# LepistaBioinformatics/blutils

Measured on AMD Instinct MI355X. Metric: Mqueries/sec consensus (synthetic outfmt-6 hit table), higher is better.
Workload: dtype i32/u32

## Files before the change

### blutils_amd/csrc/consensus_kernel.hip

```cpp

#if defined(__HIP_DEVICE_COMPILE__) && !defined(__gfx950__)
#error "consensus_kernel.hip is written for gfx950"
#endif

#include <hip/hip_runtime.h>

#include <climits>
#include <cstdint>
#include <type_traits>

#include "blu_internal.h"

namespace blu {

#define WAVE 64

constexpr int BLOCK_A = 768;
constexpr int BLU_WAVES_PER_SIMD = 3;
constexpr int BLOCK_N = 1024;
constexpr int BLU_N_WAVES_PER_SIMD = 4;
constexpr int BLOCK_F = 704;
constexpr int LIST_CAP = 208;
constexpr int LIST_CAP_RING = 248;
constexpr int LIST_CAP_F64 = 232;
// ... 681 lines not shown
                else { m[0] = wave_max_i32(m[0]); m[1] = wave_max_i32(m[1]); }
                uint32_t c[2], slot[2], tot[2], tmask[2];
#pragma unroll
                for (int hf = 0; hf < 2; ++hf) {
                    c[hf] = 0; tmask[hf] = 0;
#pragma unroll
                    for (int r = 0; r < 4; ++r) { const bool t = left[hf] > r && bs[hf][r] == m[hf]; tmask[hf] |= (uint32_t)t << r; c[hf] += (uint32_t)t; }
                    uint32_t in = c[hf];
                    in += (uint32_t)dpp<0x111>((int)in);
                    in += (uint32_t)dpp<0x112>((int)in);
                    in += (uint32_t)dpp<0x114>((int)in);
                    in += (uint32_t)dpp<0x118>((int)in);
                    const uint32_t k0 = (uint32_t)rl((int)in, 15), k1 = (uint32_t)rl((int)in, 31), k2 = (uint32_t)rl((int)in, 47), k3 = (uint32_t)rl((int)in, 63);
                    tot[hf] = k0 + k1 + k2 + k3;
                    slot[hf] = (row16 == 0 ? 0u : (row16 == 1 ? k0 : (row16 == 2 ? k0 + k1 : k0 + k1 + k2))) + in - c[hf];
                }
                const uint32_t gk = tot[0] + tot[1];
                const bool fits = fill + gk <= CAP;
                if (lane == 0) {
                    if (halves) L.meta[qi] = fits ? (fill | (gk << 16)) : META_SLOW;
                    else {
                        L.meta[qs[0]] = fits ? (fill | (tot[0] << 16)) : META_SLOW;
                        if (qs[1] < 64u) L.meta[qs[1]] = fits ? ((fill + tot[0]) | (tot[1] << 16)) : META_SLOW;
                    }
                }
                if (!fits) {
                    uint64_t rest = long_mask;
                    while (rest) { const uint32_t qn = (uint32_t)__builtin_ctzll(rest); rest &= rest - 1; if (lane == 0) L.meta[qn] = META_SLOW; }
                    break;
                }
                {
#pragma unroll
                    for (int hf = 0; hf < 2; ++hf) {
                        if (tot[hf] == 0) continue;
                        StepRegs S;
                        fetch_rest(S, voff[hf], tmask[hf]);
                        uint32_t idx = fill + (hf ? tot[0] : 0u) + slot[hf];
#pragma unroll
                        for (int r = 0; r < 4; ++r) {
                            if ((tmask[hf] >> r) & 1u) {
                                put_entry(idx, S, r, ro[hf] + sub4 + r);
                                ++idx;
                            }
                        }
                    }
                    fill += gk;
                }
            }
        };
        auto phase1_flat = [&]() {
            if constexpr (!RING) {
            constexpr uint32_t UR = FLAT_ROWS, MAXS = FLAT_STEPS, DEPTH = FLAT_DEPTH;
            static_assert(UR == 8u, "two 16-byte loads per lane");
            static_assert(FLAT_SEG >= MAX_TASK_SEG, "the flat pass takes every segment of the task");
            static_assert(DEPTH <= MAXS && MAXS * WAVE >= FLAT_SEG / UR, "a query's units fit one round");
            const uint32_t rows = L.seg[lane].y;
            const uint32_t nunit = (rows + UR - 1u) / UR;
            uint32_t incl = nunit;
            incl += (uint32_t)dpp<0x111>((int)incl);
            incl += (uint32_t)dpp<0x112>((int)incl);
            incl += (uint32_t)dpp<0x114>((int)incl);
            incl += (uint32_t)dpp<0x118>((int)incl);
            const uint32_t t0 = (uint32_t)rl((int)incl, 15), t1 = (uint32_t)rl((int)incl, 31), t2 = (uint32_t)rl((int)incl, 47);
            const uint32_t r16 = (uint32_t)lane >> 4;
            incl += r16 == 0 ? 0u : (r16 == 1 ? t0 : (r16 == 2 ? t0 + t1 : t0 + t1 + t2));
            const uint32_t q_end = incl, q_begin = incl - nunit;
            const uint64_t out_m = __ballot(rows != 0u && q_end > MAXS * WAVE);
            const uint32_t q_lim = out_m ? (uint32_t)__builtin_ctzll(out_m) : WAVE;
            const uint32_t total = q_lim < WAVE ? (uint32_t)rl((int)q_begin, (int)q_lim) : (uint32_t)rl((int)q_end, WAVE - 1);
            const uint32_t ns = (total + WAVE - 1u) / WAVE;
            L.qs[lane] = q_begin;
            L.qm[lane] = INT_MIN;
            L.qk[lane] = 0u;
            if (rows != 0u) L.meta[lane] = META_SLOW;
            __builtin_amdgcn_fence(__ATOMIC_RELEASE, "workgroup");
            __builtin_amdgcn_wave_barrier();
            __builtin_amdgcn_fence(__ATOMIC_ACQUIRE, "workgroup");
            auto issue = [&](const uint32_t st, u32x4& lo4, u32x4& hi4, uint32_t& um) {
                um = 0u;
                uint32_t voff = 0xFFFFFFF0u;
                int left = 0;
                if (st < ns) {
                    const uint32_t g = st * WAVE + (uint32_t)lane;
                    uint32_t q = 0;
#pragma unroll
                    for (uint32_t sp = 32; sp; sp >>= 1) { const uint32_t c = q + sp; if (L.qs[c] <= g) q = c; }
                    const uint2 sg = L.seg[q];
                    const uint32_t oq = g - L.qs[q];
                    left = g < total ? (int)sg.y - (int)(UR * oq) : 0;
                    if (left > 0) { voff = (sg.x + UR * oq) * 4u; um = q | (oq << 6) | (umin((uint32_t)left, UR) << 12); }
                }
                lo4 = __builtin_amdgcn_raw_buffer_load_b128(rs_bs, voff, 0, STREAM_AUX);
                hi4 = __builtin_amdgcn_raw_buffer_load_b128(rs_bs, left > 4 ? voff + 16u : 0xFFFFFFF0u, 0, STREAM_AUX);
            };
            u32x4 ba[DEPTH], bb[DEPTH];
            uint32_t um[MAXS];
            int lmx[MAXS];
#pragma unroll
            for (uint32_t st = 0; st < MAXS; ++st) { um[st] = 0u; lmx[st] = INT_MIN; }
#pragma unroll
            for (uint32_t st = 0; st < DEPTH; ++st) issue(st, ba[st], bb[st], um[st]);
#pragma unroll
            for (uint32_t st = 0; st < MAXS; ++st) {
                if (st >= ns) break;
                const u32x4 va = ba[st % DEPTH], vb = bb[st % DEPTH];
                const uint32_t left = (um[st] >> 12) & 15u;
                const uint32_t v[8] = {va.x, va.y, va.z, va.w, vb.x, vb.y, vb.z, vb.w};
                int bsv[UR], mx = INT_MIN;
#pragma unroll
                for (uint32_t r = 0; r < UR; ++r) { bsv[r] = left > r ? (int)v[r] : INT_MIN; mx = imax(mx, bsv[r]); }
                uint32_t lmask = 0;
#pragma unroll
                for (uint32_t r = 0; r < UR; ++r) lmask |= (uint32_t)(left > r && bsv[r] == mx) << r;
                um[st] |= lmask << 16;
                lmx[st] = mx;
                if (left) atomicMax(&L.qm[um[st] & 63u], mx);
                if (st + DEPTH < MAXS) issue(st + DEPTH, ba[st % DEPTH], bb[st % DEPTH], um[st + DEPTH]);
            }
            __builtin_amdgcn_fence(__ATOMIC_RELEASE, "workgroup");
            __builtin_amdgcn_wave_barrier();
            __builtin_amdgcn_fence(__ATOMIC_ACQUIRE, "workgroup");
            uint32_t running = fill, q_cut = q_lim;
#pragma unroll
            for (uint32_t st = 0; st < MAXS; ++st) {
                if (st >= ns) break;
                const uint32_t q = um[st] & 63u, oq = (um[st] >> 6) & 63u;
                const bool have = ((um[st] >> 12) & 15u) != 0u;
                const int M = L.qm[q];
                const uint32_t tmask = (have && lmx[st] == M) ? (um[st] >> 16) & 0xFFu : 0u;
                const uint32_t c = (uint32_t)__builtin_popcount(tmask);
                uint32_t in2 = c;
                in2 += (uint32_t)dpp<0x111>((int)in2);
                in2 += (uint32_t)dpp<0x112>((int)in2);
                in2 += (uint32_t)dpp<0x114>((int)in2);
                in2 += (uint32_t)dpp<0x118>((int)in2);
                const uint32_t k0 = (uint32_t)rl((int)in2, 15), k1 = (uint32_t)rl((int)in2, 31), k2 = (uint32_t)rl((int)in2, 47), k3 = (uint32_t)rl((int)in2, 63);
                in2 += r16 == 0 ? 0u : (r16 == 1 ? k0 : (r16 == 2 ? k0 + k1 : k0 + k1 + k2));
                const uint32_t idx0 = running + in2 - c;
                if (have && oq == 0u) L.meta[q] = META_SLOW | idx0;
                if (c) atomicAdd(&L.qk[q], c);
                const bool over = have && idx0 + c > CAP;
                const uint64_t over_m = __ballot(over);
                const bool room = !over && c != 0u && (over_m == 0ull || (uint32_t)lane < (uint32_t)__builtin_ctzll(over_m));
                if (room) L.rec[idx0] = make_uint4(__builtin_bitreverse32(tmask), L.seg[q].x + UR * oq, UR * oq, 0u);
                if (over_m) { q_cut = (uint32_t)rl((int)q, __builtin_ctzll(over_m)); break; }
                running += k0 + k1 + k2 + k3;
            }
            __builtin_amdgcn_fence(__ATOMIC_RELEASE, "workgroup");
            __builtin_amdgcn_wave_barrier();
            __builtin_amdgcn_fence(__ATOMIC_ACQUIRE, "workgroup");
            const uint32_t m = L.meta[lane];
            if (rows != 0u && (uint32_t)lane < q_cut) L.meta[lane] = (m & 0xFFFFu) | (L.qk[lane] << 16);
            fill = q_cut < q_lim ? (L.meta[q_cut] & 0xFFFFu) : running;
            if (q_cut < WAVE) stop_q = q_cut;
            }
        };
        auto ring_mark_landed = [&](const uint32_t upto) {
            const uint32_t m0 = (ring_landed + RING_CHUNKS - 1u) & ~(RING_CHUNKS - 1u);
            if (m0 < upto) {
                if ((uint32_t)lane < RING_PAD) L.ring[RING_ROWS + lane] = L.ring[lane];
                __builtin_amdgcn_fence(__ATOMIC_RELEASE, "workgroup");
                __builtin_amdgcn_wave_barrier();
                __builtin_amdgcn_fence(__ATOMIC_ACQUIRE, "workgroup");
            }
            ring_landed = upto;
        };
        auto ring_refill = [&]() {
            if (ring_head < ring_tail) { ring_head = ring_tail; if (ring_landed < ring_tail) ring_landed = ring_tail; }
            const uint32_t lim = ring_end < ring_tail + RING_CHUNKS ? ring_end : ring_tail + RING_CHUNKS;
            if (ring_head < lim) { ring_dma_run(rs_ring, ring_c0, ring_head, lim); ring_head = lim; }
        };
        auto phase1_scan = [&](const auto rpl_c, const auto full_c, const uint32_t LPQ) {
            constexpr uint32_t RPL = decltype(rpl_c)::value;
            constexpr bool FULL = decltype(full_c)::value;
            static_assert(RPL <= RING_PAD && RPL <= 32u, "rows per lane");
            const uint32_t QPS = WAVE / LPQ;
            const uint32_t grp = (uint32_t)lane / LPQ, sub = ((uint32_t)lane & (LPQ - 1u)) * RPL, row16 = (uint32_t)lane >> 4;
            {
                const uint32_t cs = (uint32_t)((vbase + (uint32_t)rl((int)seg_x, (int)first_q)) >> 8);
                if (cs < ring_tail) { wait_vmcnt(0u); ring_head = ring_landed = ring_tail = cs; }
            }
            for (uint32_t qb = first_q / QPS * QPS; qb < nq; qb += QPS) {
                const uint32_t r_lo = (uint32_t)rl((int)seg_x, (int)(qb < first_q ? first_q : qb));
                const uint32_t qn = qb + QPS;
                const uint32_t r_hi = qn < nq ? (uint32_t)rl((int)seg_x, (int)qn) : task_nrows;
                ring_tail = (uint32_t)((vbase + r_lo) >> 8);
                ring_refill();
                if (r_hi > r_lo) {
                    const uint32_t need = (uint32_t)((vbase + r_hi - 1u) >> 8);
                    if (need >= ring_landed) { wait_vmcnt(ring_head - 1u - need); ring_mark_landed(need + 1u); }
                }
                const uint32_t qi = qb + grp;
                const uint2 sg = L.seg[qi];
                const int left0 = (sg.y > short_seg ? 0 : (int)sg.y) - (int)sub;
                const uint32_t over = (FULL && left0 > 0 && left0 < (int)RPL) ? RPL - (uint32_t)left0 : 0u;
                const uint32_t sub_e = sub - over;
                const int left = FULL ? (left0 > 0 ? (int)RPL : 0) : left0;
                const uint32_t row0 = sg.x + sub_e;
                const uint32_t a = ((uint32_t)vbase + sg.x + sub_e) & RING_MASK;
                int b[RPL];
#pragma unroll
                for (uint32_t i = 0; i < RPL; ++i) b[i] = (int)L.ring[a + i];
                asm volatile("s_waitcnt lgkmcnt(0)" ::: "memory");
#pragma unroll
                for (uint32_t i = 0; i < RPL; ++i) asm volatile("" : "+v"(b[i]));
                if (r_hi > r_lo) { ring_tail = (uint32_t)((vbase + r_hi) >> 8); ring_refill(); }
                int M = INT_MIN;
                if constexpr (FULL) {
#pragma unroll
                    for (uint32_t i = 0; i < RPL; ++i) M = imax(M, b[i]);
                    M = left > 0 ? M : INT_MIN;
                } else {
#pragma unroll
                    for (uint32_t i = 0; i < RPL; ++i) { b[i] = (int)i < left ? b[i] : INT_MIN; M = imax(M, b[i]); }
                }
                if (LPQ >= 2) M = imax(M, dpp<0xB1>(M));
                if (LPQ >= 4) M = imax(M, dpp<0x4E>(M));
                if (LPQ >= 8) M = imax(M, dpp<0x141>(M));
                if (LPQ >= 16) M = imax(M, dpp<0x140>(M));
                uint32_t mask = tie_mask<RPL>(b, M);
                mask = left > 0 ? mask : 0u;
                if constexpr (FULL) mask &= 0xFFFFFFFFu >> (32u - RPL + over);
                const uint32_t c = (uint32_t)__builtin_popcount(mask);
                uint32_t incl = c;
                incl += (uint32_t)dpp<0x111>((int)incl);
                incl += (uint32_t)dpp<0x112>((int)incl);
                incl += (uint32_t)dpp<0x114>((int)incl);
                incl += (uint32_t)dpp<0x118>((int)incl);
                const uint32_t k0 = (uint32_t)rl((int)incl, 15), k1 = (uint32_t)rl((int)incl, 31);
                const uint32_t k2 = (uint32_t)rl((int)incl, 47), k3 = (uint32_t)rl((int)incl, 63);
                const bool fits = fill + k0 + k1 + k2 + k3 <= CAP;
                const uint32_t p1 = fill + k0, p2 = p1 + k1, p3 = p2 + k2;
                const uint32_t rbase = row16 == 0 ? fill : (row16 == 1 ? p1 : (row16 == 2 ? p2 : p3));
                uint32_t gk = c;
                if (LPQ >= 2) gk += (uint32_t)dpp<0xB1>((int)gk);
                if (LPQ >= 4) gk += (uint32_t)dpp<0x4E>((int)gk);
                if (LPQ >= 8) gk += (uint32_t)dpp<0x141>((int)gk);
                if (LPQ >= 16) gk += (uint32_t)dpp<0x140>((int)gk);
                if (PID32 && !fits) {
                    __builtin_amdgcn_s_setprio(2);
                    uint64_t BK = 0;
                    uint32_t bacc = 0, bpos = 0, brow = 0, kmin = 0xFFFFFFFFu, pmax = 0, dlo = 0xFFFFFFFFu, dhi = 0, err = 0xFFFFFFFFu;
                    auto reset = [&]() { BK = 0; bacc = 0; bpos = 0; brow = 0; kmin = 0xFFFFFFFFu; pmax = 0; dlo = 0xFFFFFFFFu; dhi = 0; err = 0xFFFFFFFFu; };
                    auto better = [&](const uint64_t K, const uint32_t acc, const uint32_t pos, const uint64_t K2, const uint32_t acc2, const uint32_t pos2) {
                        const bool gt = (K > K2) | ((K == K2) & (acc > acc2)), eq = (K == K2) & (acc == acc2);
                        return STRAT == BLU_RELAXED ? (gt | (eq & (pos > pos2))) : ((!gt & !eq) | (eq & (pos < pos2)));
                    };
                    auto take_record = [&](const u32x4 rec, const uint32_t gp, const bool on) {
                        const uint32_t len = umin(rec.x >> BLU_ROW_BITS, t.max_depth), pos = rec.x & ROW_MASK;
                        const bool unmatched = pos >= t.n_tax, bad = !unmatched && (rec.x >> BLU_ROW_BITS) == 0;
                        const uint32_t e = (gp << 8) | (bad ? (uint32_t)BLU_ST_ERR_BAD_LINEAGE : (uint32_t)BLU_ST_ERR_UNMATCHED_TAXID);
                        err = (on && (unmatched | bad)) ? umin(err, e) : err;
                        const uint32_t pm = rec.y & ((1u << KEY_PID_BITS) - 1u);
                        const uint32_t k1 = (len << KEY_PID_BITS) | pm;
                        const uint64_t K = ((uint64_t)k1 << 32) | (rec.z ^ 0x80000000u);
                        const bool take = on & ((kmin == 0xFFFFFFFFu) | better(K, rec.w, gp, BK, bacc, bpos));
                        BK = take ? K : BK; bacc = take ? rec.w : bacc; bpos = take ? gp : bpos; brow = take ? pos : brow;
                        kmin = on ? umin(kmin, k1) : kmin;
                        const uint32_t pmo = pm | ((!PACKED && rec.y >= (1u << KEY_PID_BITS)) ? 0x80000000u : 0u);
                        pmax = (on && pmo > pmax) ? pmo : pmax;
                        dlo = on ? umin(dlo, pos) : dlo;
                        dhi = (on && pos > dhi) ? pos : dhi;
                    };
                    auto load_record = [&](const uint32_t row, const bool on) {
                        u32x4 r;
                        if (PACKED) r = __builtin_amdgcn_raw_buffer_load_b128(rs_tax, on ? row * 16u : 0xFFFFFFC0u, 0, GATHER_AUX);
                        else {
                            const uint32_t o4 = on ? row * 4u : 0xFFFFFFF0u;
                            r.x = __builtin_amdgcn_raw_buffer_load_b32(rs_tax, o4, 0, GATHER_AUX);
                            r.y = __builtin_amdgcn_raw_buffer_load_b32(rs_pid, o4, 0, GATHER_AUX);
                            r.z = __builtin_amdgcn_raw_buffer_load_b32(rs_aln, o4, 0, GATHER_AUX);
                            r.w = __builtin_amdgcn_raw_buffer_load_b32(rs_acc, o4, 0, GATHER_AUX);
                        }
                        return r;
                    };
                    auto merge = [&](auto ctrl) {
                        constexpr int C = decltype(ctrl)::value;
                        const uint64_t K2 = ((uint64_t)(uint32_t)dpp<C>((int)(uint32_t)(BK >> 32)) << 32) | (uint32_t)dpp<C>((int)(uint32_t)BK);
                        const uint32_t acc2 = (uint32_t)dpp<C>((int)bacc), pos2 = (uint32_t)dpp<C>((int)bpos), row2 = (uint32_t)dpp<C>((int)brow);
                        const uint32_t kmin2 = (uint32_t)dpp<C>((int)kmin);
                        const bool take = (kmin2 != 0xFFFFFFFFu) & ((kmin == 0xFFFFFFFFu) | better(K2, acc2, pos2, BK, bacc, bpos));
                        BK = take ? K2 : BK; bacc = take ? acc2 : bacc; bpos = take ? pos2 : bpos; brow = take ? row2 : brow;
                        kmin = umin(kmin, kmin2);
                        const uint32_t pm2 = (uint32_t)dpp<C>((int)pmax); pmax = pm2 > pmax ? pm2 : pmax;
                        dlo = umin(dlo, (uint32_t)dpp<C>((int)dlo));
                        const uint32_t hi2 = (uint32_t)dpp<C>((int)dhi); dhi = hi2 > dhi ? hi2 : dhi;
                        err = umin(err, (uint32_t)dpp<C>((int)err));
                    };
                    auto deliver = [&](const int src, const bool mine) {
                        const uint32_t f_khi = (uint32_t)__builtin_amdgcn_ds_bpermute(src, (int)(uint32_t)(BK >> 32));
                        const uint32_t f_pos = (uint32_t)__builtin_amdgcn_ds_bpermute(src, (int)bpos), f_row = (uint32_t)__builtin_amdgcn_ds_bpermute(src, (int)brow);
                        const uint32_t f_kmin = (uint32_t)__builtin_amdgcn_ds_bpermute(src, (int)kmin), f_pmax = (uint32_t)__builtin_amdgcn_ds_bpermute(src, (int)pmax);
                        const uint32_t f_lo = (uint32_t)__builtin_amdgcn_ds_bpermute(src, (int)dlo), f_hi = (uint32_t)__builtin_amdgcn_ds_bpermute(src, (int)dhi);
                        const uint32_t f_err = (uint32_t)__builtin_amdgcn_ds_bpermute(src, (int)err);
                        const bool got = mine && f_kmin != 0xFFFFFFFFu;
                        const bool g_ovf = got && (f_pmax & 0x80000000u) != 0u, g_err = got && !g_ovf && f_err != 0xFFFFFFFFu, g_ok = got && !g_ovf && !g_err;
                        dn_flag = g_ovf ? 3u : (g_err ? 2u : (g_ok ? 1u : dn_flag));
                        dn_err = g_err ? (f_err & 0xFFu) : dn_err;
                        dn_pos = g_err ? (f_err >> 8) : dn_pos;
                        if constexpr (PID32) { r_pid = g_ok ? (f_khi & ((1u << KEY_PID_BITS) - 1u)) : r_pid; max_pid = g_ok ? f_pmax : max_pid; }
                        r_len = g_ok ? (f_khi >> KEY_PID_BITS) : r_len; r_row = g_ok ? f_row : r_row; r_pos = g_ok ? f_pos : r_pos;
                        minlen = g_ok ? (f_kmin >> KEY_PID_BITS) : minlen; g_lo = g_ok ? f_lo : g_lo; g_hi = g_ok ? f_hi : g_hi;
                    };
                    const uint32_t tq = (uint32_t)lane;
                    const bool mine = tq >= qb && tq < qn && tq < nq;
                    const uint32_t own0 = (mine ? tq - qb : 0u) * LPQ;
                    if (LPQ <= 4u && BLU_DENSE_Q * (k0 + k1 + k2 + k3) >= r_hi - r_lo) {
                        const uint32_t c4 = (uint32_t)lane & 3u;
#pragma nounroll
                        for (uint32_t g = 0; g < 4u; ++g) {
                            const int own = (int)((16u * g + ((uint32_t)lane >> 2)) * 4u);
                            const uint32_t o_row0 = (uint32_t)__builtin_amdgcn_ds_bpermute(own, (int)row0);
                            const uint32_t o_mask = (uint32_t)__builtin_amdgcn_ds_bpermute(own, (int)mask);
                            const uint32_t o_sub = (uint32_t)__builtin_amdgcn_ds_bpermute(own, (int)sub_e);
                            if (__ballot(o_mask != 0u) == 0ull) continue;
                            reset();
                            constexpr uint32_t NF = PACKED ? 4u : 2u;
#pragma unroll
                            for (uint32_t b0 = 0; b0 < RPL; b0 += 4u * NF) {
                                if (__ballot(((o_mask >> (RPL - 4u * NF - b0)) & ((1u << (4u * NF)) - 1u)) != 0u) == 0ull) continue;
                                u32x4 rq[NF];
#pragma unroll
                                for (uint32_t j = 0; j < NF; ++j) {
                                    const uint32_t i = b0 + 4u * j + c4;
                                    rq[j] = load_record(o_row0 + i, ((o_mask >> (RPL - 1u - i)) & 1u) != 0u);
                                }
#pragma unroll
                                for (uint32_t j = 0; j < NF; ++j) {
                                    const uint32_t i = b0 + 4u * j + c4;
                                    take_record(rq[j], o_sub + i, ((o_mask >> (RPL - 1u - i)) & 1u) != 0u);
                                }
                            }
                            merge(std::integral_constant<int, 0xB1>());
                            merge(std::integral_constant<int, 0x4E>());
                            if (LPQ >= 2) merge(std::integral_constant<int, 0x141>());
                            if (LPQ >= 4) merge(std::integral_constant<int, 0x140>());
                            deliver((int)(((own0 & 15u) * 4u) * 4u), mine && (own0 >> 4) == g);
                        }
                    } else {
                        uint32_t m = mask;
                        while (__ballot(m != 0u)) {
                            u32x4 rq[4];
                            uint32_t gp[4];
#pragma unroll
                            for (int j = 0; j < 4; ++j) {
                                const bool on = m != 0u;
                                const uint32_t hb = on ? 31u - (uint32_t)__builtin_clz(m) : 0u, i = RPL - 1u - hb;
                                m = on ? (m & ~(1u << hb)) : 0u;
                                gp[j] = on ? sub_e + i : 0xFFFFFFFFu;
                                rq[j] = load_record(row0 + i, on);
                            }
#pragma unroll
                            for (int j = 0; j < 4; ++j) take_record(rq[j], gp[j], gp[j] != 0xFFFFFFFFu);
                        }
                        if (LPQ >= 2) merge(std::integral_constant<int, 0xB1>());
                        if (LPQ >= 4) merge(std::integral_constant<int, 0x4E>());
                        if (LPQ >= 8) merge(std::integral_constant<int, 0x141>());
                        if (LPQ >= 16) merge(std::integral_constant<int, 0x140>());
                        deliver((int)(own0 * 4u), mine);
                    }
                    {
                        const uint32_t f_gk = (uint32_t)__builtin_amdgcn_ds_bpermute((int)(own0 * 4u), (int)gk);
                        dn_k = (mine && dn_flag == 1u) ? f_gk : dn_k;
                    }
                    if (sub == 0 && gk != 0u) L.meta[qi] = META_DENSE;
                    __builtin_amdgcn_s_setprio(0);
                    continue;
                }
                uint32_t idx = rbase + incl - c;
                if (!fits) {
                    const uint32_t lane_o = (uint32_t)__builtin_ctzll(__ballot(idx + c > CAP));
                    const uint32_t qo = qb + lane_o / LPQ;
                    const bool taken = qi < qo;
                    if (sub == 0) L.meta[qi] = taken ? (idx | (gk << 16)) : META_SLOW;
                    if (taken && c) { L.rec[idx].x = mask << (32u - RPL); L.rec[idx].y = DESC_WORD1(RPL, row0, sub_e); }
                    fill = (uint32_t)rl((int)idx, (int)((qo - qb) * LPQ));
                    stop_q = qo;
                    wait_vmcnt(0u);
                    ring_head = ring_landed = ring_tail = (uint32_t)((vbase + (uint32_t)rl((int)seg_x, (int)qo)) >> 8);
                    break;
                }
                if (sub == 0) L.meta[qi] = idx | (gk << 16);
                fill = p3 + k3;
                static_assert((RPL == 16u || RPL == 32u) && SHORT_SEG <= 128u, "descriptor word of a lane");
                if (c) { L.rec[idx].x = mask << (32u - RPL); L.rec[idx].y = DESC_WORD1(RPL, row0, sub_e); }
            }
        };
        auto gather_list = [&](auto&& between) {
            constexpr int NG = (CAP + WAVE - 1) / WAVE;
            u32x4 g[NG];
            uint32_t ghi[NG], gpos[NG], ghint[NG];
            uint32_t carry = 0;
#pragma unroll
            for (int u = 0; u < NG; ++u) {
                g[u] = u32x4{0u, 0u, 0u, 0u}; ghi[u] = 0u; gpos[u] = 0u; ghint[u] = 0u;
                if ((uint32_t)u * WAVE >= fill_ring) continue;
                const uint32_t idx = (uint32_t)u * WAVE + (uint32_t)lane;
                const bool valid = idx < fill_ring;
                const uint32_t d0 = L.rec[idx < CAP ? idx : 0u].x;
                int s = (valid && d0 != 0u) ? (int)idx : 0;
                s = imax(s, dpp<0x111>(s));
                s = imax(s, dpp<0x112>(s));
                s = imax(s, dpp<0x114>(s));
                s = imax(s, dpp<0x118>(s));
                s = imax(s, __builtin_amdgcn_update_dpp(0, s, 0x142, 0xA, 0xF, false));
                s = imax(s, __builtin_amdgcn_update_dpp(0, s, 0x143, 0xC, 0xF, false));
                s = imax(s, (int)carry);
                carry = (uint32_t)rl(s, 63);
                const uint4 dd = L.rec[s];
                const uint32_t d0w = dd.x, d = dd.y;
                uint32_t r = idx - (uint32_t)s, x = scan_rpl == 32u ? d0w : d0w >> 16, i = 0;
                if (scan_rpl == 32u) {
                    const uint32_t h = x >> 16, ch = (uint32_t)__builtin_popcount(h);
                    const bool low = r >= ch;
                    r -= low ? ch : 0u; x = low ? (x & 0xFFFFu) : h; i += low ? 16u : 0u;
                }
                {
                    const uint32_t h = x >> 8, ch = (uint32_t)__builtin_popcount(h);
                    const bool low = r >= ch;
                    r -= low ? ch : 0u; x = low ? (x & 0xFFu) : h; i += low ? 8u : 0u;
                }
                {
                    const uint32_t h = x >> 4, ch = (uint32_t)__builtin_popcount(h);
                    const bool low = r >= ch;
                    r -= low ? ch : 0u; x = low ? (x & 0xFu) : h; i += low ? 4u : 0u;
                }
                {
                    const uint32_t h = x >> 2, ch = (uint32_t)__builtin_popcount(h);
                    const bool low = r >= ch;
                    r -= low ? ch : 0u; x = low ? (x & 0x3u) : h; i += low ? 2u : 0u;
                }
                i += (r >= (x >> 1)) ? 1u : 0u;
                const uint32_t row = (RING ? (d >> DESC_SUB_BITS) : d) + i;
                gpos[u] = (RING ? (d & ((1u << DESC_SUB_BITS) - 1u)) : dd.z) + i;
                if (PACKED) g[u] = __builtin_amdgcn_raw_buffer_load_b128(rs_tax, valid ? row * 16u : 0xFFFFFFC0u, 0, GATHER_AUX);
                else if (WIDE) {
                    g[u] = __builtin_amdgcn_raw_buffer_load_b128(rs_tax, valid ? row * 24u : 0xFFFFFFC0u, 0, GATHER_AUX);
                    const u32x2 p = __builtin_amdgcn_raw_buffer_load_b64(rs_tax, valid ? row * 24u + 16u : 0xFFFFFFE0u, 0, GATHER_AUX);
                    ghint[u] = g[u].y;
                    g[u].y = p.x; ghi[u] = p.y;
                } else {
                    const uint32_t o4 = valid ? row * 4u : 0xFFFFFFF0u;
                    g[u].x = __builtin_amdgcn_raw_buffer_load_b32(rs_tax, o4, 0, GATHER_AUX);
                    if (PID32) g[u].y = __builtin_amdgcn_raw_buffer_load_b32(rs_pid, o4, 0, GATHER_AUX);
                    else {
                        const u32x2 p = __builtin_amdgcn_raw_buffer_load_b64(rs_pid, valid ? row * 8u : 0xFFFFFFE0u, 0, GATHER_AUX);
                        g[u].y = p.x; ghi[u] = p.y;
                    }
                    g[u].z = __builtin_amdgcn_raw_buffer_load_b32(rs_aln, o4, 0, GATHER_AUX);
                    g[u].w = __builtin_amdgcn_raw_buffer_load_b32(rs_acc, o4, 0, GATHER_AUX);
                }
            }
            between();
            bool ovf = false;
            uint32_t gk[NG];
#pragma unroll
            for (int u = 0; u < NG; ++u) {
                const bool valid = (uint32_t)u * WAVE + (uint32_t)lane < fill_ring;
                if constexpr (PID32) { gk[u] = g[u].y & PM_MASK; ovf |= !PACKED && valid && g[u].y >= (1u << KEY_PID_BITS); }
                else {
                    const double p = __hiloint2double((int)ghi[u], (int)g[u].y);
                    const bool in_range = p >= 0.0 && p < 131.0705;
                    const uint32_t k = in_range ? (uint32_t)(p * 1000.0 + 0.5) : 0u;
                    const double back = milli17_to_f64(k);
                    gk[u] = k;
                    ovf |= valid && !(in_range && __double2hiint(back) == (int)ghi[u] && __double2loint(back) == (int)g[u].y && k < BLU_KTHR_NEVER);
                }
            }
            keyed = __ballot(ovf) == 0ull && fill == fill_ring;
            bool any_bad = false;
#pragma unroll
            for (int u = 0; u < NG; ++u) {
                const uint32_t idx = (uint32_t)u * WAVE + (uint32_t)lane;
                if (idx < fill_ring) {
                    if (keyed) {
                        const uint32_t len = umin(g[u].x >> BLU_ROW_BITS, t.max_depth);
                        any_bad |= len == 0u || (g[u].x & ROW_MASK) >= t.n_tax;
                        const uint32_t hint = (PID32 ? g[u].y : ghint[u]) >> KEY_PID_BITS;
                        L.rec[idx] = make_uint4((g[u].x & ROW_MASK) | ((hint >> 8) << BLU_ROW_BITS),
                                                (len << KEYED_LEN_SHIFT) | (gk[u] << KEYED_PID_SHIFT) | (hint & 0xFFu), g[u].z ^ 0x80000000u, g[u].w);
                    } else L.rec[idx] = make_uint4(g[u].x, g[u].y, g[u].z, g[u].w);
                    L.pq[idx] = (uint16_t)gpos[u];
                    if (!PID32) L.p1[idx] = ghi[u];
                }
            }
            keyed_bad = __ballot(any_bad) != 0ull;
        };
        bool pend = (uint32_t)lane < nq;
        uint32_t pend_before = WAVE + 1;
        if (RING && contiguous) {
            ring_c0 = (uint32_t)(vbase >> 8);
            rs_ring = ring_desc(ring_c0);
            ring_end = task_nrows ? (uint32_t)((vbase + task_nrows - 1u) >> 8) + 1u : ring_c0;
            if (pref_q0 != q0_32) ring_head = ring_landed = ring_c0;
            ring_tail = ring_c0;
        }
        for (;;) {
        fill = 0;
        stop_q = WAVE;
        bool ring_round = false;
        bool list_round = false;
        keyed = false;
        {
            const uint32_t rows = L.seg[lane].y;
            const uint64_t live = __ballot(rows != 0u);
            first_q = live ? (uint32_t)__builtin_ctzll(live) : 0u;
            {
                const uint32_t n16 = (uint32_t)__builtin_popcountll(__ballot(rows != 0u && rows <= 16u));
                const uint32_t n32 = (uint32_t)__builtin_popcountll(__ballot(rows != 0u && rows <= 32u));
                const uint32_t n64 = (uint32_t)__builtin_popcountll(__ballot(rows != 0u && rows <= 64u));
                const uint32_t n128 = (uint32_t)__builtin_popcountll(__ballot(rows != 0u && rows <= SHORT_SEG));
                const uint32_t c16 = 4u * n16 + BLU_LONG_COST * (n128 - n16), c32 = 8u * n32 + BLU_LONG_COST * (n128 - n32);
                const uint32_t c64 = 16u * n64 + BLU_LONG_COST * (n128 - n64), c128 = 32u * n128;
                uint32_t best = c128;
                short_seg = SHORT_SEG;
                if (c64 < best) { best = c64; short_seg = 64u; }
                if (c32 < best) { best = c32; short_seg = 32u; }
                if (c16 < best) { best = c16; short_seg = 16u; }
            }
            bool flat_round = false;
            if constexpr (!RING) {
                const uint32_t n128 = (uint32_t)__builtin_popcountll(__ballot(rows != 0u && rows <= SHORT_SEG));
                const uint32_t n_over = (uint32_t)__builtin_popcountll(__ballot(rows > SHORT_SEG));
                uint32_t best;
                {
                    const uint32_t n16 = (uint32_t)__builtin_popcountll(__ballot(rows != 0u && rows <= 16u));
                    const uint32_t n32 = (uint32_t)__builtin_popcountll(__ballot(rows != 0u && rows <= 32u));
                    const uint32_t n64 = (uint32_t)__builtin_popcountll(__ballot(rows != 0u && rows <= 64u));
                    best = 32u * n128;
                    best = umin(best, 16u * n64 + BLU_LONG_COST * (n128 - n64));
                    best = umin(best, 8u * n32 + BLU_LONG_COST * (n128 - n32));
                    best = umin(best, 4u * n16 + BLU_LONG_COST * (n128 - n16));
                }
                const uint32_t units = (uint32_t)wave_sum_u32((rows + FLAT_ROWS - 1u) / FLAT_ROWS);
                flat_round = units != 0u && units + units / 4u + 64u < best + BLU_LONG_COST * n_over;
                if (flat_round) { short_seg = FLAT_SEG; scan_rpl = 16u; }
            }
            const uint32_t longest = flat_round ? 0u : wave_max_u32(rows > short_seg ? 0u : rows);
            ring_round = RING && contiguous && longest != 0u && all_short && __ballot(rows > short_seg) == 0ull;
            uint32_t lpq = 1;
            if (ring_round) {
                scan_rpl = longest > 32u ? 32u : 16u;
                while (lpq * scan_rpl < longest) lpq *= 2;
                while ((WAVE / lpq) * longest + 256u > RING_ROWS) lpq *= 2;
            }
            list_round = ring_round || flat_round;
            if (list_round) {
#pragma unroll
                for (uint32_t u = 0; u * WAVE < CAP; ++u) { const uint32_t i = u * WAVE + (uint32_t)lane; if (i < CAP) L.rec[i].x = 0u; }
            }
            if (ring_round) {
                const bool all_full = __ballot(rows != 0u && rows <= short_seg && rows < scan_rpl) == 0ull;
                if (scan_rpl == 32u) {
                    if (all_full) phase1_scan(std::integral_constant<uint32_t, 32>(), std::true_type(), lpq);
                    else phase1_scan(std::integral_constant<uint32_t, 32>(), std::false_type(), lpq);
                } else phase1_scan(std::integral_constant<uint32_t, 16>(), std::false_type(), lpq);
            }
            else if (flat_round) phase1_flat();
            else if (longest > 32u && longest <= 64u) phase1(std::integral_constant<uint32_t, 16>(), false);
            else if (longest) phase1(longest <= 16u ? 4u : (longest <= 32u ? 8u : 32u), longest >= (PACKED ? 9u : 25u));
            if (stop_q < WAVE && rows != 0u && ((uint32_t)lane >= stop_q || rows > short_seg)) L.meta[lane] = META_SLOW;
            fill_ring = list_round ? fill : 0u;
            const uint64_t long_mask = __ballot(rows > short_seg);
            if (long_mask && stop_q == WAVE) phase1_long(long_mask);
        }
        __builtin_amdgcn_fence(__ATOMIC_RELEASE, "workgroup");
        __builtin_amdgcn_wave_barrier();
        __builtin_amdgcn_fence(__ATOMIC_ACQUIRE, "workgroup");
        const bool last_round = __ballot(pend && (my_end - my_off) != 0u && (my_end - my_off) <= MAX_TASK_SEG && in_span && (L.meta[lane] & META_SLOW)) == 0ull;
        uint32_t nxt_c0 = 0, nxt_lim = 0;
        if (RING && last_round && nx_nq != 0u) {
            uint32_t n_off = nx_off, n_end = nx_end;
            asm volatile("" : "+v"(n_off), "+v"(n_end));
            if (n_end > n_hits32) n_end = n_hits32;
            if (n_off > n_end) n_off = n_end;
            const uint32_t nqn = nx_nq;
            const uint32_t n_start = (uint32_t)rl((int)n_off, 0);
            const bool n_span = n_off >= n_start && (n_end - n_start) <= (uint32_t)TASK_SPAN;
            const uint32_t rel_end = n_end - n_start, rel_off = n_off - n_start;
            const uint32_t prev_end = (uint32_t)__shfl_up((int)rel_end, 1);
            const bool ok = n_span && (n_end - n_off) <= SHORT_SEG && (lane == 0 || rel_off == prev_end);
            const uint32_t n_rows = (uint32_t)rl((int)rel_end, (int)nqn - 1);
            if (__ballot((uint32_t)lane < nqn && !ok) == 0ull && n_rows != 0u) {
                const uint64_t vb = (uint64_t)n_start + mis;
                nxt_c0 = (uint32_t)(vb >> 8);
                const uint32_t cend = (uint32_t)((vb + n_rows - 1u) >> 8) + 1u;
                nxt_lim = cend < nxt_c0 + RING_CHUNKS ? cend : nxt_c0 + RING_CHUNKS;
            }
        }
        auto prefetch_next = [&]() {
            if (nxt_lim > nxt_c0) {
                const auto rsn = ring_desc(nxt_c0);
                ring_dma_run(rsn, nxt_c0, nxt_c0, nxt_lim);
                ring_head = nxt_lim; ring_landed = nxt_c0; ring_tail = nxt_c0;
                pref_q0 = nx_q0;
            }
        };
        __builtin_amdgcn_s_setprio(3);
        if (list_round) gather_list(prefetch_next);
        else prefetch_next();
        __builtin_amdgcn_fence(__ATOMIC_RELEASE, "workgroup");
        __builtin_amdgcn_wave_barrier();
        __builtin_amdgcn_fence(__ATOMIC_ACQUIRE, "workgroup");

        {
            const uint32_t nrows = my_end - my_off;
            const uint32_t m = L.meta[lane];
            const bool listed = pend && nrows != 0 && nrows <= MAX_TASK_SEG && in_span && !(m & (META_SLOW | META_DENSE));
            const uint32_t first = listed ? (m & 0xFFFFu) : 0u, k = listed ? ((m >> 16) & 0x3FFu) : 0u;
            const uint32_t kmax = wave_max_u32(k);
            uint32_t err = 0, err_pos = 0, nan_pos = 0xFFFFFFFFu;
            uint32_t b_len = 0, b_acc = 0, lo = 0xFFFFFFFFu, hi = 0, l_minlen = 0xFFFFFFFFu, l_row = 0, l_pos = 0, l_hint = 0;
            int b_aln = 0;
            PK b_pid = 0, l_maxpid = 0;
            const uint32_t last_e = k ? k - 1u : 0u;
            uint4 nx_rec = make_uint4(0, 0, 0, 0);
            uint32_t nx_pq = 0;
            uint32_t l_keyed = 0;
            if (!keyed) { nx_rec = L.rec[first]; nx_pq = L.pq[first]; }
            if (keyed) {
                l_keyed = 1u;
                uint64_t BK = 0;
                uint32_t kmin = 0xFFFFFFFFu, pmax = 0;
                uint32_t l_idx = first;
                auto step = [&](const auto check_c, const uint4 x, const uint32_t xidx, const bool is_first) {
                    const uint32_t pos = x.x & ROW_MASK;
                    if constexpr (decltype(check_c)::value) {
                        const bool unmatched = pos >= t.n_tax, bad = x.y < (1u << KEYED_LEN_SHIFT);
                        const bool first_err = (err == 0) & (unmatched | bad);
                        err = first_err ? (unmatched ? (uint32_t)BLU_ST_ERR_UNMATCHED_TAXID : (uint32_t)BLU_ST_ERR_BAD_LINEAGE) : err;
                        err_pos = first_err ? (uint32_t)L.pq[xidx] : err_pos;
                    }
                    kmin = umin(kmin, x.y);
                    lo = umin(lo, pos);
                    hi = pos > hi ? pos : hi;
                    const uint32_t ky = x.y & ~0xFFu;
                    const uint32_t pm = (x.y >> KEYED_PID_SHIFT) & PM_MASK;
                    pmax = pm > pmax ? pm : pmax;
                    const uint64_t K = ((uint64_t)ky << 32) | x.z;
                    const bool gt = (K > BK) | ((K == BK) & (x.w > b_acc)), eq = (K == BK) & (x.w == b_acc);
                    const bool take = is_first | (STRAT == BLU_RELAXED ? (gt | eq) : !(gt | eq));
                    BK = take ? K : BK;
                    b_acc = take ? x.w : b_acc;
                    l_idx = take ? xidx : l_idx;
                };
                auto reduce = [&](const auto check_c) {
                    for (uint32_t e = 0; e < kmax; e += 4) {
                        uint4 x[4];
                        uint32_t xi[4];
#pragma unroll
                        for (uint32_t j = 0; j < 4; ++j) {
                            xi[j] = first + (e + j < k ? e + j : last_e);
                            x[j] = L.rec[xi[j]];
                        }
#pragma unroll
                        for (uint32_t j = 0; j < 4; ++j) step(check_c, x[j], xi[j], e == 0 && j == 0);
                    }
                };
                if (keyed_bad) reduce(std::true_type()); else reduce(std::false_type());
                const uint32_t l_x = L.rec[l_idx].x, l_y = L.rec[l_idx].y;
                l_pos = L.pq[l_idx];
                const uint32_t k1 = (uint32_t)(BK >> 32);
                b_len = k1 >> KEYED_LEN_SHIFT;
                l_minlen = kmin >> KEYED_LEN_SHIFT;
                l_row = l_x & ROW_MASK;
                l_hint = ((l_x >> BLU_ROW_BITS) << 8) | (l_y & 0xFFu);
// ... 711 lines not shown
```

Baseline: 11610.

## Balance record loads across lane pairs and pack descriptor shuffles in consensus

In the sparse per-query path, each lane splits its record mask with its neighbour lane using a prefix-xor parity trick, so both lanes of a pair take records from the combined mask. Loads per iteration also rise from 4 to 6, with positions packed as bytes to save registers. In the dense path, row and sub-offset are sent as one packed descriptor word, which removes one bpermute per group. The dense load batch for the non-packed layout is widened, and the mine/own0 values become recomputed lambdas to ease register pressure. The extra registers for rq[6] could lower occupancy.

```diff
diff --git a/blutils_amd/csrc/consensus_kernel.hip b/blutils_amd/csrc/consensus_kernel.hip
--- a/blutils_amd/csrc/consensus_kernel.hip
+++ b/blutils_amd/csrc/consensus_kernel.hip
@@ -1007,66 +1007,86 @@
                         r_len = g_ok ? (f_khi >> KEY_PID_BITS) : r_len; r_row = g_ok ? f_row : r_row; r_pos = g_ok ? f_pos : r_pos;
                         minlen = g_ok ? (f_kmin >> KEY_PID_BITS) : minlen; g_lo = g_ok ? f_lo : g_lo; g_hi = g_ok ? f_hi : g_hi;
                     };
-                    const uint32_t tq = (uint32_t)lane;
-                    const bool mine = tq >= qb && tq < qn && tq < nq;
-                    const uint32_t own0 = (mine ? tq - qb : 0u) * LPQ;
+                    auto q_mine = [&]() { const uint32_t tq = (uint32_t)lane; return tq >= qb && tq < qn && tq < nq; };
+                    auto q_own0 = [&]() { return (q_mine() ? (uint32_t)lane - qb : 0u) * LPQ; };
                     if (LPQ <= 4u && BLU_DENSE_Q * (k0 + k1 + k2 + k3) >= r_hi - r_lo) {
                         const uint32_t c4 = (uint32_t)lane & 3u;
+                        const uint32_t w_me = DESC_WORD1(RPL, row0, sub_e);
 #pragma nounroll
                         for (uint32_t g = 0; g < 4u; ++g) {
                             const int own = (int)((16u * g + ((uint32_t)lane >> 2)) * 4u);
-                            const uint32_t o_row0 = (uint32_t)__builtin_amdgcn_ds_bpermute(own, (int)row0);
+                            const uint32_t o_w = (uint32_t)__builtin_amdgcn_ds_bpermute(own, (int)w_me);
                             const uint32_t o_mask = (uint32_t)__builtin_amdgcn_ds_bpermute(own, (int)mask);
-                            const uint32_t o_sub = (uint32_t)__builtin_amdgcn_ds_bpermute(own, (int)sub_e);
                             if (__ballot(o_mask != 0u) == 0ull) continue;
                             reset();
-                            constexpr uint32_t NF = PACKED ? 4u : 2u;
+                            constexpr uint32_t NF_LAYOUT = PACKED ? 4u : 4u;
+                            constexpr uint32_t NF = 4u * NF_LAYOUT > RPL ? RPL / 4u : NF_LAYOUT;
+                            constexpr uint32_t BATCH_BITS = 4u * NF == 32u ? 0xFFFFFFFFu : (1u << (4u * NF)) - 1u;
 #pragma unroll
                             for (uint32_t b0 = 0; b0 < RPL; b0 += 4u * NF) {
-                                if (__ballot(((o_mask >> (RPL - 4u * NF - b0)) & ((1u << (4u * NF)) - 1u)) != 0u) == 0ull) continue;
+                                if (__ballot(((o_mask >> (RPL - 4u * NF - b0)) & BATCH_BITS) != 0u) == 0ull) continue;
                                 u32x4 rq[NF];
 #pragma unroll
                                 for (uint32_t j = 0; j < NF; ++j) {
                                     const uint32_t i = b0 + 4u * j + c4;
-                                    rq[j] = load_record(o_row0 + i, ((o_mask >> (RPL - 1u - i)) & 1u) != 0u);
+                                    rq[j] = load_record((o_w >> DESC_SUB_BITS) + i, ((o_mask >> (RPL - 1u - i)) & 1u) != 0u);
                                 }
 #pragma unroll
                                 for (uint32_t j = 0; j < NF; ++j) {
                                     const uint32_t i = b0 + 4u * j + c4;
-                                    take_record(rq[j], o_sub + i, ((o_mask >> (RPL - 1u - i)) & 1u) != 0u);
+                                    take_record(rq[j], (o_w & ((1u << DESC_SUB_BITS) - 1u)) + i, ((o_mask >> (RPL - 1u - i)) & 1u) != 0u);
                                 }
                             }
                             merge(std::integral_constant<int, 0xB1>());
                             merge(std::integral_constant<int, 0x4E>());
                             if (LPQ >= 2) merge(std::integral_constant<int, 0x141>());
                             if (LPQ >= 4) merge(std::integral_constant<int, 0x140>());
-                            deliver((int)(((own0 & 15u) * 4u) * 4u), mine && (own0 >> 4) == g);
+                            deliver((int)(((q_own0() & 15u) * 4u) * 4u), q_mine() && (q_own0() >> 4) == g);
                         }
                     } else {
-                        uint32_t m = mask;
-                        while (__ballot(m != 0u)) {
-                            u32x4 rq[4];
-                            uint32_t gp[4];
-#pragma unroll
-                            for (int j = 0; j < 4; ++j) {
-                                const bool on = m != 0u;
-                                const uint32_t hb = on ? 31u - (uint32_t)__builtin_clz(m) : 0u, i = RPL - 1u - hb;
-                                m = on ? (m & ~(1u << hb)) : 0u;
-                                gp[j] = on ? sub_e + i : 0xFFFFFFFFu;
-                                rq[j] = load_record(row0 + i, on);
+                        constexpr uint32_t NF_OWN = PACKED ? 6u : 6u;
+                        static_assert(SHORT_SEG <= 128u && DESC_SUB_BITS == 8u, "a position in the segment is a byte, 0xFF = no record");
+                        const uint32_t w_own = DESC_WORD1(RPL, row0, sub_e);
+                        uint32_t m = mask, mp = 0u, w_par = 0u;
+                        if (LPQ >= 2u) {
+                            uint32_t px = mask;
+                            px ^= px << 1; px ^= px << 2; px ^= px << 4; px ^= px << 8; px ^= px << 16;
+                            m = mask & px;
+                            mp = (uint32_t)dpp<0xB1>((int)(mask & ~px));
+                            w_par = (uint32_t)dpp<0xB1>((int)w_own);
+                        }
+                        while (__ballot((m | mp) != 0u)) {
+                            u32x4 rq[NF_OWN];
+                            uint32_t gp[(NF_OWN + 3u) / 4u];
+#pragma unroll
+                            for (uint32_t j = 0; j < (NF_OWN + 3u) / 4u; ++j) gp[j] = 0xFFFFFFFFu;
+#pragma unroll
+                            for (uint32_t j = 0; j < NF_OWN; ++j) {
+                                const bool own = m != 0u, on = (m | mp) != 0u;
+                                const uint32_t src = own ? m : mp, w = own ? w_own : w_par;
+                                const uint32_t hb = on ? 31u - (uint32_t)__builtin_clz(src) : 0u, i = RPL - 1u - hb;
+                                const uint32_t keep = ~(1u << hb);
+                                m = own ? (m & keep) : m;
+                                mp = own ? mp : (mp & keep);
+                                const uint32_t pos = on ? (w & 0xFFu) + i : 0xFFu;
+                                gp[j / 4u] ^= (pos ^ 0xFFu) << (8u * (j & 3u));
+                                rq[j] = load_record((w >> DESC_SUB_BITS) + i, on);
                             }
 #pragma unroll
-                            for (int j = 0; j < 4; ++j) take_record(rq[j], gp[j], gp[j] != 0xFFFFFFFFu);
+                            for (uint32_t j = 0; j < NF_OWN; ++j) {
+                                const uint32_t pos = (gp[j / 4u] >> (8u * (j & 3u))) & 0xFFu;
+                                take_record(rq[j], pos, pos != 0xFFu);
+                            }
                         }
                         if (LPQ >= 2) merge(std::integral_constant<int, 0xB1>());
                         if (LPQ >= 4) merge(std::integral_constant<int, 0x4E>());
                         if (LPQ >= 8) merge(std::integral_constant<int, 0x141>());
                         if (LPQ >= 16) merge(std::integral_constant<int, 0x140>());
-                        deliver((int)(own0 * 4u), mine);
+                        deliver((int)(q_own0() * 4u), q_mine());
                     }
                     {
-                        const uint32_t f_gk = (uint32_t)__builtin_amdgcn_ds_bpermute((int)(own0 * 4u), (int)gk);
-                        dn_k = (mine && dn_flag == 1u) ? f_gk : dn_k;
+                        const uint32_t f_gk = (uint32_t)__builtin_amdgcn_ds_bpermute((int)(q_own0() * 4u), (int)gk);
+                        dn_k = (q_mine() && dn_flag == 1u) ? f_gk : dn_k;
                     }
                     if (sub == 0 && gk != 0u) L.meta[qi] = META_DENSE;
                     __builtin_amdgcn_s_setprio(0);
```

Measured after the change: 10730. 0.924x the previous value.
